# Fanchuana/OPUS-PLLM

Measured on AMD Instinct MI355X. Metric: proteins_per_sec, higher is better.
Workload: dtype f16; 1 GPU; OPUS-PLLM-llama3_8b shape: batch 64/GPU, 512-residue proteins, 89-id prompt (+8 protein tokens = 96 positions), 32 new tokens, greedy (BASELINE configs[3] per-GPU shard: batch 512 over 8 GPUs); batch_per_gpu=64, residues=512, parallelism=replicas x1 (batch-sharded), all-gather of ids

## Files before the change

### opus-pllm_amd/csrc/attn_prefill.hip

```cpp
#include "common.h"
#include <type_traits>

namespace opus {

constexpr int KB = 64;

template <int HDP>
__device__ __forceinline__ int kswz(int row, int chunk) {
    if (HDP == 128) return chunk ^ (row & 15);
    if (HDP == 64) return chunk ^ ((row >> 1) & 7);
    return chunk;
}
template <int HD>
__device__ __forceinline__ int vswz(int row) {
    if (HD == 128) return (row & 7) << 1;
    if (HD == 64) return ((row >> 1) & 3) << 1;
    if (HD == 32) return ((row >> 2) & 1) << 1;
    return 0;
}

typedef float f2 __attribute__((ext_vector_type(2)));
__device__ __forceinline__ float max3(float a, float b, float c) {
    float r;
    asm("v_max3_f32 %0, %1, %2, %3" : "=v"(r) : "v"(a), "v"(b), "v"(c));
    return r;
}
__device__ __forceinline__ float xor16_max(float x) {
    float a = x, b = x, r;
    asm volatile("s_nop 1\n\tv_permlane16_swap_b32 %0, %1" : "+v"(a), "+v"(b));
    asm("v_max_f32 %0, %1, %2" : "=v"(r) : "v"(a), "v"(b));
    return r;
}
__device__ __forceinline__ void xor32_pair(float x, float &a, float &b) {
    a = x;
    b = x;
    asm volatile("s_nop 1\n\tv_permlane32_swap_b32 %0, %1" : "+v"(a), "+v"(b));
}

typedef short s4v __attribute__((ext_vector_type(4)));
typedef short s8v __attribute__((ext_vector_type(8)));

template <int HD, bool CAUSAL, int QT>
__global__ __launch_bounds__(256) void attn_prefill_kernel(AttnParams p) {
    constexpr int QW = 16 * QT, QB = 4 * QW;
    constexpr int HDP = HD < 32 ? 32 : HD;
    constexpr int KS = HDP / 32;
    constexpr int NO = HD / 16;
    constexpr int CH = HDP / 8;
    constexpr int VC = HD / 8;
    __shared__ __attribute__((aligned(16))) half_t sK[2][KB * HDP];
    __shared__ __attribute__((aligned(16))) half_t sV[2][KB * HD];

    const int tid = threadIdx.x, lane = tid & 63;
    const int wave = __builtin_amdgcn_readfirstlane(tid >> 6);
    const int g = lane >> 4, li = lane & 15;
    const int qtrim = (p.q_trim && p.cu) ? 1 : 0;
    const int nqb = (p.T - 2 * qtrim + QB - 1) / QB;
    const int id = blockIdx.x, slot = id >> 3;
    const int bh = (slot / nqb) * 8 + (id & 7);
    if (bh >= p.B * p.heads) return;
    const int b = bh / p.heads, h = bh % p.heads, hk = h / p.group;
    const int q0 = (slot % nqb) * QB + qtrim, qw = q0 + wave * QW;
    int T = p.T, Tq = p.T;
    int64_t qb_off = (int64_t)b * p.q_sb, kb_off = (int64_t)b * p.k_sb, vb_off = (int64_t)b * p.v_sb, ob_off = (int64_t)b * p.o_sb;
    if (p.cu) {
        const int r0 = p.cu[b];
        T = p.cu[b + 1] - r0;
        Tq = T - qtrim;
        if (q0 >= Tq) return;
        qb_off = (int64_t)r0 * p.q_st; kb_off = (int64_t)r0 * p.k_st; vb_off = (int64_t)r0 * p.v_st; ob_off = (int64_t)r0 * p.o_st;
    }
    const int kstart = (p.kstart && !p.cu) ? p.kstart[b] : 0;
    const int kend = (p.kend && !p.cu) ? p.kend[b] : T;

    const half_t *Qb = p.Q + qb_off + (int64_t)h * HD;
    const half_t *Kb = p.K + kb_off + (int64_t)hk * HD;
    const half_t *Vb = p.V + vb_off + (int64_t)hk * HD;

    h8 qf[QT][KS];
#pragma unroll
    for (int t = 0; t < QT; ++t) {
        int qr = qw + 16 * t + li;
        qr = qr < Tq ? qr : Tq - 1;
        const half_t *src = Qb + (int64_t)qr * p.q_st;
#pragma unroll
        for (int s = 0; s < KS; ++s) {
            const int d = 32 * s + 8 * g;
            qf[t][s] = d < HD ? *reinterpret_cast<const h8 *>(src + d) : h8{0, 0, 0, 0, 0, 0, 0, 0};
        }
    }
    f4 o[QT][NO];
    float mrow[QT], lrow[QT];
#pragma unroll
    for (int t = 0; t < QT; ++t) {
        mrow[t] = -INFINITY;
        lrow[t] = 0.f;
#pragma unroll
        for (int n = 0; n < NO; ++n) o[t][n] = f4{0.f, 0.f, 0.f, 0.f};
    }

    int k_lo = kstart / KB * KB;
    int k_hi = kend;
    if (CAUSAL) {
        const int last_q = (q0 + QB - 1 < T - 1 ? q0 + QB - 1 : T - 1);
        k_hi = k_hi < last_q + 1 ? k_hi : last_q + 1;
    }
    const float sc = p.scale * 1.4426950408889634f;
    const bool wave_live = qw < Tq;

    constexpr int KL = KB * CH / 256;
    constexpr int VN = KB * VC;
    constexpr int VL = VN >= 256 ? VN / 256 : 1;
    static_assert(KL >= 1, "tile too small for 256 threads");
    h8 kreg[KL], vreg[VL];
    const __amdgpu_buffer_rsrc_t krs = __builtin_amdgcn_make_buffer_rsrc((void *)Kb, 0, (int)(((int64_t)(T - 1) * p.k_st + HD) * 2), 0x00020000);
    const __amdgpu_buffer_rsrc_t vrs = __builtin_amdgcn_make_buffer_rsrc((void *)Vb, 0, (int)(((int64_t)(T - 1) * p.v_st + HD) * 2), 0x00020000);
    int koff[KL], voff[VL];
#pragma unroll
    for (int u = 0; u < KL; ++u) {
        const int i = tid + 256 * u, r = i / CH, c = i % CH;
        koff[u] = c * 8 < HD ? (int)((r * p.k_st + c * 8) * 2) : 0x7ffffff0;
    }
#pragma unroll
    for (int u = 0; u < VL; ++u) {
        const int i = tid + 256 * u, r = i / VC, c = i % VC;
        voff[u] = i < VN ? (int)((r * p.v_st + c * 8) * 2) : 0x7ffffff0;
    }
    auto load_tile = [&](int kt) {
        const int kb = kt * (int)p.k_st * 2, vb = kt * (int)p.v_st * 2;
#pragma unroll
        for (int u = 0; u < KL; ++u) kreg[u] = __builtin_bit_cast(h8, __builtin_amdgcn_raw_buffer_load_b128(krs, koff[u] + kb, 0, 0));
#pragma unroll
        for (int u = 0; u < VL; ++u) vreg[u] = __builtin_bit_cast(h8, __builtin_amdgcn_raw_buffer_load_b128(vrs, voff[u] + vb, 0, 0));
    };
    auto store_tile = [&](int buf) {
#pragma unroll
        for (int u = 0; u < KL; ++u) {
            const int i = tid + 256 * u, r = i / CH, c = i % CH;
            *reinterpret_cast<h8 *>(&sK[buf][r * HDP + kswz<HDP>(r, c) * 8]) = kreg[u];
        }
#pragma unroll
        for (int u = 0; u < VL; ++u) {
            const int i = tid + 256 * u, r = i / VC, c = i % VC;
            if (i < VN) *reinterpret_cast<h8 *>(&sV[buf][r * HD + (c ^ vswz<HD>(r)) * 8]) = vreg[u];
        }
    };

    if (k_lo < k_hi) {
        load_tile(k_lo);
        store_tile(0);
        if (k_lo + KB < k_hi) load_tile(k_lo + KB);
    }
    __syncthreads();
    auto tile_body = [&](auto nsub_tag, int kt, int buf) {
        {
            constexpr int NSUB = decltype(nsub_tag)::value, NJ = (NSUB + 1) / 2;
            const half_t *tK = sK[buf], *tV = sV[buf];
            f4 s[QT][4];
#pragma unroll
            for (int n = 0; n < NSUB; ++n) {
                const int r = 16 * n + li;
                h8 kf[KS];
#pragma unroll
                for (int ks = 0; ks < KS; ++ks) kf[ks] = *reinterpret_cast<const h8 *>(tK + r * HDP + kswz<HDP>(r, 4 * ks + g) * 8);
#pragma unroll
                for (int t = 0; t < QT; ++t) {
                    s[t][n] = f4{0.f, 0.f, 0.f, 0.f};
#pragma unroll
                    for (int ks = 0; ks < KS; ++ks) s[t][n] = mfma16(kf[ks], qf[t][ks], s[t][n]);
                }
            }
            const bool interior = kt >= kstart && kt + KB <= kend && (!CAUSAL || kt + KB - 1 <= qw);
            if (__builtin_expect(!interior, 0)) {
#pragma unroll
                for (int t = 0; t < QT; ++t) {
                    const int qi = qw + 16 * t + li;
#pragma unroll
                    for (int n = 0; n < NSUB; ++n)
#pragma unroll
                        for (int r = 0; r < 4; ++r) {
                            const int kj = kt + 16 * n + 4 * g + r;
                            bool vis = kj >= kstart && kj < kend;
                            if (CAUSAL) vis = vis && kj <= qi;
                            s[t][n][r] = vis ? s[t][n][r] : -INFINITY;
                        }
                }
            }
            h8 pf[QT][2];
#pragma unroll
            for (int t = 0; t < QT; ++t) {
                float mx = fmaxf(fmaxf(s[t][0][0], s[t][0][1]), fmaxf(s[t][0][2], s[t][0][3]));
#pragma unroll
                for (int n = 1; n < NSUB; ++n) mx = fmaxf(fmaxf(mx, fmaxf(s[t][n][0], s[t][n][1])), fmaxf(s[t][n][2], s[t][n][3]));
                float ma, mb;
                mx = xor16_max(mx);
                xor32_pair(mx, ma, mb);
                const float mnew = max3(mrow[t], ma, mb);
                const float msafe = mnew == -INFINITY ? 0.f : mnew;
                const float msc = msafe * sc;
                if (!__all(mnew == mrow[t])) {
                    const float alpha = __builtin_amdgcn_exp2f((mrow[t] - msafe) * sc);
                    lrow[t] *= alpha;
#pragma unroll
                    for (int n = 0; n < NO; ++n) o[t][n] *= alpha;
                    mrow[t] = mnew;
                }
                const f2 sc2 = f2{sc, sc}, msc2 = f2{msc, msc};
                f2 rs2 = f2{0.f, 0.f};
#pragma unroll
                for (int n = 0; n < NSUB; ++n)
#pragma unroll
                    for (int r = 0; r < 4; r += 2) {
                        const f2 a = f2{s[t][n][r], s[t][n][r + 1]} * sc2 - msc2;
                        const f2 e = f2{__builtin_amdgcn_exp2f(a[0]), __builtin_amdgcn_exp2f(a[1])};
                        s[t][n][r] = e[0];
                        s[t][n][r + 1] = e[1];
                        rs2 += e;
                    }
                lrow[t] += rs2[0] + rs2[1];
#pragma unroll
                for (int j = 0; j < NJ; ++j) {
                    const bool two = 2 * j + 1 < NSUB;
                    pf[t][j] = h8{(half_t)s[t][2 * j][0], (half_t)s[t][2 * j][1], (half_t)s[t][2 * j][2], (half_t)s[t][2 * j][3],
                                  two ? (half_t)s[t][two ? 2 * j + 1 : 0][0] : (half_t)0.f, two ? (half_t)s[t][two ? 2 * j + 1 : 0][1] : (half_t)0.f,
                                  two ? (half_t)s[t][two ? 2 * j + 1 : 0][2] : (half_t)0.f, two ? (half_t)s[t][two ? 2 * j + 1 : 0][3] : (half_t)0.f};
                }
            }
#pragma unroll
            for (int n = 0; n < NO; ++n)
#pragma unroll
                for (int j = 0; j < NJ; ++j) {
                    const int r0 = 16 * (2 * j) + 4 * g + (li >> 2), r1 = r0 + 16;
                    const int cc = 2 * n + ((li & 3) >> 1), off = (li & 1) * 4;
                    const s4v lo = __builtin_amdgcn_ds_read_tr16_b64_v4i16(
                        (__attribute__((address_space(3))) s4v *)(tV + r0 * HD + (cc ^ vswz<HD>(r0)) * 8 + off));
                    const s4v hi = __builtin_amdgcn_ds_read_tr16_b64_v4i16(
                        (__attribute__((address_space(3))) s4v *)(tV + r1 * HD + (cc ^ vswz<HD>(r1)) * 8 + off));
                    const s8v both = s8v{lo[0], lo[1], lo[2], lo[3], hi[0], hi[1], hi[2], hi[3]};
                    const h8 vf = __builtin_bit_cast(h8, both);
#pragma unroll
                    for (int t = 0; t < QT; ++t) o[t][n] = mfma16(vf, pf[t][j], o[t][n]);
                }
        }
    };
    auto run = [&](auto live_tag) {
        constexpr bool LIVE = decltype(live_tag)::value;
        int kt = k_lo, buf = 0;
        for (; k_hi - kt > 32; kt += KB, buf ^= 1) {
            if constexpr (LIVE) tile_body(std::integral_constant<int, 4>{}, kt, buf);
            if (kt + KB < k_hi) {
                store_tile(buf ^ 1);
                if (kt + 2 * KB < k_hi) load_tile(kt + 2 * KB);
            }
            __syncthreads();
        }
        if constexpr (LIVE) {
            if (kt < k_hi) {
                if (k_hi - kt > 16) tile_body(std::integral_constant<int, 2>{}, kt, buf);
                else tile_body(std::integral_constant<int, 1>{}, kt, buf);
            }
        }
    };
    if (wave_live) run(std::true_type{});
    else run(std::false_type{});

    if (!wave_live) return;
#pragma unroll
    for (int t = 0; t < QT; ++t) {
        float l = lrow[t];
        l += __shfl_xor(l, 16, 64);
        l += __shfl_xor(l, 32, 64);
        const int qi = qw + 16 * t + li;
        if (qi >= Tq) continue;
        const float inv = l > 0.f ? 1.0f / l : 0.f;
        half_t *dst = p.O + ob_off + (int64_t)qi * p.o_st + (int64_t)h * HD;
#pragma unroll
        for (int n = 0; n < NO; ++n)
            *reinterpret_cast<h4 *>(dst + 16 * n + 4 * g) =
                h4{(half_t)(o[t][n][0] * inv), (half_t)(o[t][n][1] * inv), (half_t)(o[t][n][2] * inv), (half_t)(o[t][n][3] * inv)};
    }
}

template <int HD, int QT>
static hipError_t launch_qt(const AttnParams &p, hipStream_t s) {
    const int nqb = cdiv(p.T - ((p.q_trim && p.cu) ? 2 : 0), 64 * QT);
    dim3 grid(((p.B * p.heads + 7) / 8) * 8 * nqb);
    if (p.causal) OPUS_LAUNCH(KC_ATTN_PREFILL, (attn_prefill_kernel<HD, true, QT>), grid, dim3(256), 0, s, p);
    else OPUS_LAUNCH(KC_ATTN_PREFILL, (attn_prefill_kernel<HD, false, QT>), grid, dim3(256), 0, s, p);
    return hipGetLastError();
}
int attn_prefill_query_tiles(const AttnParams &p) {
    bool one = !(p.head_dim <= 64 && (int64_t)p.B * p.heads * cdiv(p.T, 128) >= 512);
    if (g_knobs.misc[3]) one = !one;
    return one ? 1 : 2;
}
template <int HD>
static hipError_t launch_hd(const AttnParams &p, hipStream_t s) {
    return attn_prefill_query_tiles(p) == 1 ? launch_qt<HD, 1>(p, s) : launch_qt<HD, 2>(p, s);
}

hipError_t launch_attn_prefill(const AttnParams &p, hipStream_t s) {
    if (p.T <= 0 || p.B <= 0) return hipErrorInvalidValue;
    if ((p.o_st & 3) || (p.o_sb & 3) || (p.q_st & 7) || (p.k_st & 7) || (p.v_st & 7) || (p.q_sb & 7) || (p.k_sb & 7) || (p.v_sb & 7))
        return hipErrorInvalidValue;
    if ((int64_t)p.T * (p.k_st > p.v_st ? p.k_st : p.v_st) * 2 >= (1ll << 31)) return hipErrorInvalidValue;
    switch (p.head_dim) {
        case 16: return launch_hd<16>(p, s);
        case 32: return launch_hd<32>(p, s);
        case 64: return launch_hd<64>(p, s);
        case 128: return launch_hd<128>(p, s);
    }
    return hipErrorInvalidValue;
}

}
```

Measured before the change: 259.3 proteins/s.

## Stage attention prefill K/V tiles via buffer-load-to-LDS DMA

Adds a DMA variant of the prefill attention kernel that loads K/V tiles straight into LDS with buffer_load ... lds. Swizzling moves into the global source offsets, and the loop changes to a wait, barrier, then issue-next-tile schedule. This removes the register staging and the ds_write stores, and lowers register pressure (occupancy hint of 4 for HD64/QT2). The trade-off is an exposed wait of vmcnt(0) at every tile, and correctness depends on M0 handling and the swizzled layout matching.

New measurement: 259.5 proteins/s (median of 2 runs). Within noise of the previous version (+0.1%).

```diff
diff --git a/opus-pllm_amd/csrc/attn_prefill.hip b/opus-pllm_amd/csrc/attn_prefill.hip
--- a/opus-pllm_amd/csrc/attn_prefill.hip
+++ b/opus-pllm_amd/csrc/attn_prefill.hip
@@ -37,11 +37,18 @@
     asm volatile("s_nop 1\n\tv_permlane32_swap_b32 %0, %1" : "+v"(a), "+v"(b));
 }
 
+__device__ __forceinline__ void dma_piece(u32x4 rs, unsigned lds, int voff) {
+    unsigned keep;
+    asm volatile("s_mov_b32 %0, m0\n\ts_mov_b32 m0, %1\n\ts_nop 0\n\tbuffer_load_dwordx4 %2, %3, 0 offen lds\n\ts_mov_b32 m0, %0"
+                 : "=&s"(keep) : "s"(lds), "v"(voff), "s"(rs) : "memory");
+}
+
 typedef short s4v __attribute__((ext_vector_type(4)));
 typedef short s8v __attribute__((ext_vector_type(8)));
 
-template <int HD, bool CAUSAL, int QT>
-__global__ __launch_bounds__(256) void attn_prefill_kernel(AttnParams p) {
+template <int HD, bool CAUSAL, int QT, bool DMA>
+__global__ __launch_bounds__(256, DMA && HD == 64 && QT == 2 ? 4 : 1) void attn_prefill_kernel(AttnParams p) {
+    static_assert(!DMA || HD >= 64, "LDS-DMA staging: whole 1-KB pieces only");
     constexpr int QW = 16 * QT, QB = 4 * QW;
     constexpr int HDP = HD < 32 ? 32 : HD;
     constexpr int KS = HDP / 32;
@@ -118,12 +125,12 @@
     int koff[KL], voff[VL];
 #pragma unroll
     for (int u = 0; u < KL; ++u) {
-        const int i = tid + 256 * u, r = i / CH, c = i % CH;
+        const int i = tid + 256 * u, r = i / CH, c = DMA ? kswz<HDP>(r, i % CH) : i % CH;
         koff[u] = c * 8 < HD ? (int)((r * p.k_st + c * 8) * 2) : 0x7ffffff0;
     }
 #pragma unroll
     for (int u = 0; u < VL; ++u) {
-        const int i = tid + 256 * u, r = i / VC, c = i % VC;
+        const int i = tid + 256 * u, r = i / VC, c = DMA ? (i % VC) ^ vswz<HD>(r) : i % VC;
         voff[u] = i < VN ? (int)((r * p.v_st + c * 8) * 2) : 0x7ffffff0;
     }
     auto load_tile = [&](int kt) {
@@ -132,6 +139,23 @@
         for (int u = 0; u < KL; ++u) kreg[u] = __builtin_bit_cast(h8, __builtin_amdgcn_raw_buffer_load_b128(krs, koff[u] + kb, 0, 0));
 #pragma unroll
         for (int u = 0; u < VL; ++u) vreg[u] = __builtin_bit_cast(h8, __builtin_amdgcn_raw_buffer_load_b128(vrs, voff[u] + vb, 0, 0));
+    };
+    const uint64_t kaddr = (uint64_t)Kb, vaddr = (uint64_t)Vb;
+    const u32x4 krw = u32x4{(unsigned)kaddr, (unsigned)(kaddr >> 32) & 0xffffu, (unsigned)(((int64_t)(T - 1) * p.k_st + HD) * 2), 0x00020000u};
+    const u32x4 vrw = u32x4{(unsigned)vaddr, (unsigned)(vaddr >> 32) & 0xffffu, (unsigned)(((int64_t)(T - 1) * p.v_st + HD) * 2), 0x00020000u};
+    const unsigned ldsK = (unsigned)(uintptr_t)(__attribute__((address_space(3))) half_t *)&sK[0][0];
+    const unsigned ldsV = (unsigned)(uintptr_t)(__attribute__((address_space(3))) half_t *)&sV[0][0];
+    auto dma_tile = [&](int kt, int buf) {
+        const int kb = kt * (int)p.k_st * 2, vb = kt * (int)p.v_st * 2;
+#pragma unroll
+        for (int u = 0; u < KL; ++u) dma_piece(krw, ldsK + (buf * KB * HDP + (wave * 64 + 256 * u) * 8) * 2, koff[u] + kb);
+#pragma unroll
+        for (int u = 0; u < VL; ++u) dma_piece(vrw, ldsV + (buf * KB * HD + (wave * 64 + 256 * u) * 8) * 2, voff[u] + vb);
+    };
+    auto publish = [&](int kt, int buf) {
+        asm volatile("s_waitcnt vmcnt(0) lgkmcnt(0)" ::: "memory");
+        __builtin_amdgcn_s_barrier();
+        if (kt + KB < k_hi) dma_tile(kt + KB, buf ^ 1);
     };
     auto store_tile = [&](int buf) {
 #pragma unroll
@@ -146,12 +170,20 @@
         }
     };
 
-    if (k_lo < k_hi) {
-        load_tile(k_lo);
-        store_tile(0);
-        if (k_lo + KB < k_hi) load_tile(k_lo + KB);
-    }
-    __syncthreads();
+    if constexpr (DMA) {
+        if (k_lo < k_hi) dma_tile(k_lo, 0);
+#pragma unroll
+        for (int t = 0; t < QT; ++t)
+#pragma unroll
+            for (int s = 0; s < KS; ++s) asm volatile("" : "+v"(qf[t][s]));
+    } else {
+        if (k_lo < k_hi) {
+            load_tile(k_lo);
+            store_tile(0);
+            if (k_lo + KB < k_hi) load_tile(k_lo + KB);
+        }
+        __syncthreads();
+    }
     auto tile_body = [&](auto nsub_tag, int kt, int buf) {
         {
             constexpr int NSUB = decltype(nsub_tag)::value, NJ = (NSUB + 1) / 2;
@@ -246,6 +278,20 @@
     auto run = [&](auto live_tag) {
         constexpr bool LIVE = decltype(live_tag)::value;
         int kt = k_lo, buf = 0;
+        if constexpr (DMA) {
+            for (; k_hi - kt > (LIVE ? 32 : 0); kt += KB, buf ^= 1) {
+                publish(kt, buf);
+                if constexpr (LIVE) tile_body(std::integral_constant<int, 4>{}, kt, buf);
+            }
+            if constexpr (LIVE) {
+                if (kt < k_hi) {
+                    publish(kt, buf);
+                    if (k_hi - kt > 16) tile_body(std::integral_constant<int, 2>{}, kt, buf);
+                    else tile_body(std::integral_constant<int, 1>{}, kt, buf);
+                }
+            }
+            return;
+        }
         for (; k_hi - kt > 32; kt += KB, buf ^= 1) {
             if constexpr (LIVE) tile_body(std::integral_constant<int, 4>{}, kt, buf);
             if (kt + KB < k_hi) {
@@ -285,8 +331,15 @@
 static hipError_t launch_qt(const AttnParams &p, hipStream_t s) {
     const int nqb = cdiv(p.T - ((p.q_trim && p.cu) ? 2 : 0), 64 * QT);
     dim3 grid(((p.B * p.heads + 7) / 8) * 8 * nqb);
-    if (p.causal) OPUS_LAUNCH(KC_ATTN_PREFILL, (attn_prefill_kernel<HD, true, QT>), grid, dim3(256), 0, s, p);
-    else OPUS_LAUNCH(KC_ATTN_PREFILL, (attn_prefill_kernel<HD, false, QT>), grid, dim3(256), 0, s, p);
+    if constexpr (HD >= 64) {
+        if (!g_knobs.misc[2]) {
+            if (p.causal) OPUS_LAUNCH(KC_ATTN_PREFILL, (attn_prefill_kernel<HD, true, QT, true>), grid, dim3(256), 0, s, p);
+            else OPUS_LAUNCH(KC_ATTN_PREFILL, (attn_prefill_kernel<HD, false, QT, true>), grid, dim3(256), 0, s, p);
+            return hipGetLastError();
+        }
+    }
+    if (p.causal) OPUS_LAUNCH(KC_ATTN_PREFILL, (attn_prefill_kernel<HD, true, QT, false>), grid, dim3(256), 0, s, p);
+    else OPUS_LAUNCH(KC_ATTN_PREFILL, (attn_prefill_kernel<HD, false, QT, false>), grid, dim3(256), 0, s, p);
     return hipGetLastError();
 }
 int attn_prefill_query_tiles(const AttnParams &p) {
```
